# hypre-space/hypredrive

Hardware: AMD Instinct MI355X
Metric: DOF/s, AMG-PCG solve phase, 3D 7-pt Laplacian (higher is better)
Workload: dtype f64

## Files before the change

### hypredrive_amd/_lib.py

```python
import ctypes as C
import os

import numpy as np

_HERE = os.path.dirname(os.path.abspath(__file__))
_LIBPATH = os.path.join(_HERE, "lib", "libhypredrv_amd.so")
_L = None


class LibraryError(RuntimeError):
    pass


class AmgParams(C.Structure):
    _fields_ = [("coarsen_type", C.c_int), ("interp_type", C.c_int), ("pmax", C.c_int),
                ("trunc_factor", C.c_double), ("strong_th", C.c_double),
                ("max_row_sum", C.c_double), ("max_coarse_size", C.c_int),
                ("min_coarse_size", C.c_int), ("max_levels", C.c_int),
                ("relax_down", C.c_int), ("relax_up", C.c_int), ("relax_coarse", C.c_int),
                ("sweeps_down", C.c_int), ("sweeps_up", C.c_int), ("sweeps_coarse", C.c_int),
                ("relax_weight", C.c_double), ("outer_weight", C.c_double),
                ("seed", C.c_uint64), ("num_functions", C.c_int),
                ("cheby_order", C.c_int), ("cheby_eig_est", C.c_int), ("cheby_variant", C.c_int), ("cheby_scale", C.c_int),
                ("cheby_fraction", C.c_double),
# ... 94 lines not shown
        "hda_mgr_blk_inverses": (I, [VP, I, I, DP, IP, IP]),
        "hda_amg_num_levels": (I, [VP]), "hda_amg_level_matrix": (I, [VP, I, I, OUT]), "hda_amg_level_cf": (I, [VP, I, IP]),
        "hda_amg_fold_sweep": (I, [VP, I, DP, DP, DP, DP, DP]), "hda_amg_blocks": (I, [VP]), "hda_amg_level_blocks": (I, [VP, I, LP]),
        "hda_amg_complexities": (I, [VP, DP, DP]), "hda_amg_vcycle_bytes": (D, [VP]), "hda_amg_vcycle": (I, [VP, DP, DP]),
        "hda_pcg": krylov, "hda_gmres": krylov, "hda_fgmres": krylov, "hda_bicgstab": krylov,
        "hda_spmm": (I, [VP, I, I, D, D, DP, DP, DP, DP, DP, DP, DP]), "hda_multi_blas": (I, [I, I, I, DP, DP, IP, DP, DP, DP, DP, DP]),
        "hda_amg_vcycle_multi": (I, [VP, I, DP, DP]), "hda_pcg_multi": (I, [VP, VP, KRY, I, DP, DP, DP, IP, IP, DP]),
        "hda_time_kernel_multi": (I, [I, VP, VP, I, I, DP, DP]),
        "hda_time_kernel": (I, [I, VP, VP, I, DP, DP]), "hda_set_overlap": (None, [I]), "hda_last_precond_calls": (I, []),
        "hda_solve_device": (I, [VP, VP, KRY, I, DP, I, DP, IP, DP, DP, DP, DP]),
        "hda_pcg_iteration_bytes": (D, [VP]), "hda_format_bytes": (I, [VP, VP, DP, DP, DP, IP]),
        "hda_csr_form": (I, [VP, I, IP]), "hda_spmv_mode": (I, [VP, I, I, D, D, DP, DP, DP, DP, DP, DP, DP, DP, DP, IP]),
        "hda_borrow_hypredrv": (I, [VP, OUT, OUT]), "hda_amd_partitioned_levels": (I, [VP]), "hda_amd_hierarchy_levels": (I, [VP]),
        "hda_halo_plan_host": (I, [I, LLP, LLP, I, IP, IP, IP, I, IP]),
        "hda_dev_alloc": (I, [I64, OUT]), "hda_dev_free": (I, [VP]), "hda_dev_upload": (I, [VP, VP, I64]),
        "hda_dev_download": (I, [VP, VP, I64]), "hda_borrow_ij_matrix": (I, [VP, OUT]), "hda_ij_ghost_gids": (I, [VP, LLP, I, IP]),
        "hda_ij_last_assembly": (I, [DP]),
        "hda_probe_spmv": (I, [VP, I]), "hda_probe_read": (I, [DP, IP]), "hda_probe_add": (I, [VP, I, IP]),
        "hda_probe_read_id": (I, [I, DP, IP]),
        "hda_comm_stats": (I, [DP, I]), "hda_comm_name": (S, []), "hda_comm_size": (I, []), "hda_comm_selftest": (I, []),
        "hda_check_row_total": (I, [C.c_longlong, I]),
        "hda_memory_stats": (I, [DP, DP]), "hda_memory_cached": (D, []), "hda_memory_driver_stats": (I, [DP, I]), "hda_memory_trim": (I, []),
    }
    undeclared = {"hda_amg_rebind": (I, [VP, VP]), "hda_amg_level0_sweep": (I, [VP, I, DP, DP, DP, DP, IP])}
    return declared, undeclared


_DECLARED, _UNDECLARED = _signatures()
SYMBOLS = list(_DECLARED)


TESTRANKS_SYMBOLS = ["hda_thread_ranks_lap7", "hda_thread_world_create", "hda_thread_world_join", "hda_thread_world_leave",
                     "hda_thread_world_destroy", "hda_testranks_selftest"]
_TESTRANKS_PATH = os.path.join(os.path.dirname(_LIBPATH), "libhypredrv_amd_testranks.so")
_T = None


def load_testranks():
    global _T
    if _T is None:
        load()
        if not os.path.exists(_TESTRANKS_PATH):
            raise LibraryError(f"{_TESTRANKS_PATH} not built: run `python -c 'import __graft_entry__ as g; g.build()'`")
        _T = C.CDLL(_TESTRANKS_PATH)
    return _T


# ... 348 lines not shown
    def blocks(self):
        return load().hda_amg_blocks(self.h)

    def level_blocks(self, level):
        out = np.zeros(max(self.blocks, 1) + 1, dtype=np.int64)
        _check(load().hda_amg_level_blocks(self.h, level, out.ctypes.data_as(C.POINTER(C.c_int64))))
        return out

    @property
    def complexities(self):
        g, o = C.c_double(), C.c_double()
        _check(load().hda_amg_complexities(self.h, C.byref(g), C.byref(o)))
        return g.value, o.value

    @property
    def vcycle_bytes(self):
        return load().hda_amg_vcycle_bytes(self.h)

    def vcycle(self, b):
        b = np.ascontiguousarray(b, dtype=np.float64)
        x = np.zeros_like(b)
        _check(load().hda_amg_vcycle(self.h, _dp(b), _dp(x)))
        return x

    def vcycle_multi(self, B):
        B = _cols(B)
        k = B.shape[1]
        bt = np.ascontiguousarray(B.T)
        xt = np.zeros_like(bt)
        _check(load().hda_amg_vcycle_multi(self.h, k, _dp(bt), _dp(xt)))
        return xt.T.copy()


MGR_INTERP = {"injection": 0, "l1-jacobi": 1, "jacobi": 2, "blk-jacobi": 12}
MGR_COARSE = {"rap": 0, "galerkin": 0, "non-galerkin": 1}
MGR_RESTRICT = {"injection": 0, "jacobi": 2, "columped": 14}
MGR_FRELAX = {"jacobi": 7, "single": 7, "l1-jacobi": 18, "amg": 2, "ilu": 32}
MGR_GRELAX = {"none": -1, "h-fgs": 3, "h-bgs": 4, "h-ssor": 6, "l1-hfgs": 13, "l1-hbgs": 14, "l1-hsgs": 88, "ilu": 16}

MGR_KRYLOV = {"pcg": 1, "gmres": 2, "fgmres": 3, "bicgstab": 4}


def _mgr_nested(entry, lv):
    for key, pre in (("f_krylov", "frelax"), ("coarsest_krylov", "coarse")):
        nk = lv.get(key)
        if not nk:
# ... 585 lines not shown
```

### hypredrive_amd/csrc/hda_amg.h

```cpp
#pragma once

#include "hda_dist.h"
#include "hda_kernels.h"

#include <chrono>
#include <memory>
#include <string>
#include <vector>

namespace hda {

struct IluParams {
   int tri_solve = 1;
   int lower_it = 5, upper_it = 5;
   int max_iter = 1;
   int                    blocks = 1;
   std::vector<long long> block_part;
};

struct AmgParams {
   int    coarsen_type    = 8;
   double strong_th       = 0.25;
   double max_row_sum     = 0.9;
   int    max_coarse_size = 64;
// ... 180 lines not shown
 public:
   void        setup(const DCsr &A, const FsaiParams &p, const std::vector<int> *part = nullptr);
   void        apply(const double *r, double *z);
   const DCsr &factor() const { return G; }
   const DCsr &factor_t() const { return GT; }
   double      apply_bytes() const;
   FsaiParams  prm;
   int         n = 0, nblocks = 1, fallback_rows = 0;
   int         class_rows[5] = {0, 0, 0, 0, 0};
   double      omega = 1.0;
   double      setup_ms[4] = {0, 0, 0, 0};

 private:
   DCsr           G, GT;
   DArray<double> work;
};

struct FirstSweepFusion {
   bool          valid = false;
   const double *dinv  = nullptr;
   const unsigned char *rclass = nullptr;
   const double *cdinv = nullptr;
   double       *dest  = nullptr;
   int           n     = 0;
   const void   *owner = nullptr;
   bool          done  = false;
   const double *in    = nullptr;
   double       *out   = nullptr;
};
FirstSweepFusion &first_sweep_fusion();

struct AmgLevel {
   DCsr           A, P, R;
   DCsr           Pt;
   bool           folded = false;
   DCsr           Pg;
   bool           pg_ready = false;
   GsPlan         gs;
   std::unique_ptr<Ilu> ilu;
   std::unique_ptr<Fsai> fsai;
   bool complex_smoother() const { return ilu || fsai; }
   DArray<double> cheb_ds, cheb_v, cheb_w;
   double         cheb_coef[5] = {0, 0, 0, 0, 0}, cheb_max_eig = 0.0, cheb_min_eig = 0.0;
   DArray<double> ilu_r, ilu_c;
   DArray<int>    cf;
   std::vector<int> blk_part;
   DArray<double> dinv_down, dinv_up;
   DArray<double> cdinv_down, cdinv_up;
   unsigned long long cdinv_gen = 0;
   DArray<double> dinv_pts[2][2];
   TwoStage       ts;
// ... 29 lines not shown
   void apply(const double *b, double *x, int dot_slot = -1);
   void apply_offering(const double *b, double *x, int dot_slot = -1);
   bool first_sweep_fusable() const;
   double *first_sweep_dest(double *x);
   void solve(const double *b, double *x);
   void        apply_multi(const double *B, double *X, int K);
   std::string multi_cycle_refusal() const;
   double      vcycle_multi_bytes(int K) const;

   int           num_levels() const { return (int)levels.size(); }
   const DCsr   &level_A(int l) const { return l == 0 ? *A0 : levels[l].A; }
   AmgLevel     &level(int l) { return levels[l]; }
   double        operator_complexity() const;
   double        grid_complexity() const;
   double        vcycle_bytes(bool format = false) const;
   bool          level_folded(int l) const { return l >= 0 && l < num_levels() && levels[(size_t)l].folded; }
   bool          level0_sweep(int dir, const double *b, const double *x, double *out, int dot_slot);
   AmgParams     prm;
   int           blocks_used = 1;
   const std::vector<int> &level_blocks(int l) const { return levels[(size_t)l].blk_part; }
   double        setup_times[8] = {0};

 private:
   void cycle(const double *b, double *x, bool zero_guess, int dot_slot, bool first_sweep_given = false);
   void relax(int l, int type, const double *dinv, const double *b, double *&cur, double *&alt,
              bool zero_guess, int dot_slot);
   int           sweep_points(int dir, int s) const;
   const double *sweep_dinv(int l, int dir, int s);
   void          build_class_dinv();
   const double *class_dinv(int l, const double *dinv);
   void          check_air_params() const;
   bool          needs_cf_in_cycle() const;
   void build_hierarchy(const DCsr &A, bool keep_ap = false);
   void build_smoother_data(int l);
   bool fold_level(int l);
   void build_cheby(int l);
   void cheby_sweep(int l, const double *b, double *u, bool zero_guess, bool ghosts_fresh = false);
   bool ghosts_fresh_ = false;
   void coarse_solve(const double *f, double *u);
   const HaloPlan &level_hA(int l) const { return (l == 0 && hA0) ? *hA0 : levels[l].hA; }
   const DCsr           *A0 = nullptr;
   int                   a0_dims[3] = {0, 0, 0};
   const HaloPlan       *hA0 = nullptr;
   bool                  dist = false;
   long long             coarse_lo = 0;
   int                   coarse_nloc = 0;
   double                stats_nnz[32] = {0}, stats_rows[32] = {0};
// ... 192 lines not shown
```

### hypredrive_amd/csrc/hda_amg_setup.hip

```cpp
#include "hda_amg.h"
#include "hda_sort.h"


#include <algorithm>
#include <chrono>
#include <cstring>

namespace hda {

#define STREAM (Context::get().stream)

void exclusive_scan64(long n, const int *in, long long *out);


__global__ __launch_bounds__(256) void k_strength(int n, const int *__restrict__ rp,
                                                  const int *__restrict__ cj,
                                                  const double *__restrict__ v, double theta,
                                                  double mrs, unsigned char *__restrict__ smask,
                                                  int *__restrict__ ns, const int *__restrict__ dof)
{
   const int i = blockIdx.x * 256 + threadIdx.x;
   if (i >= n) return;
   const int k0 = rp[i], k1 = rp[i + 1];
   double    diag = 0.0, row_sum = 0.0, row_scale = 0.0;
// ... 3583 lines not shown

FirstSweepFusion &first_sweep_fusion()
{
   return RankState<FirstSweepFusion>::get();
}
bool Amg::first_sweep_fusable() const
{
   const char *e = getenv("HDA_FUSE_Z0");
   return !(e && atoi(e) == 0) && num_levels() > 1 && prm.sweeps_down >= 1 && is_jacobi_type(prm.relax_down) && !levels[0].complex_smoother();
}
double *Amg::first_sweep_dest(double *x)
{
   auto oop = [&](int t) { return is_jacobi_type(t) || (levels[0].gs.nblk > 0 && (t == 3 || t == 4 || t == 13 || t == 14)); };
   const int swaps0 = levels[0].complex_smoother() ? 0 : (oop(prm.relax_down) ? (prm.sweeps_down - (prm.sweeps_down > 0 ? 1 : 0)) : 0) +
                                             (oop(prm.relax_up) ? prm.sweeps_up : 0);
   return (swaps0 & 1) ? levels[0].u2.data() : x;
}
void Amg::apply_offering(const double *b, double *x, int dot_slot)
{
   FirstSweepFusion &fs = first_sweep_fusion();
   const bool given = fs.done && fs.owner == this && fs.in == b && fs.out == x;
   fs.done          = false;
   HDA_REQUIRE(!given || first_sweep_fusable(), "first sweep handed to a cycle that does not open with one");
   cycle(b, x, true, dot_slot, given);
   fs.valid = first_sweep_fusable();
   if (fs.valid)
   {
      double *d = first_sweep_dest(x);
      fs.dinv   = sweep_dinv(0, 0, 0);
      fs.cdinv  = class_dinv(0, fs.dinv);
      fs.rclass = fs.cdinv ? row_classes(level_A(0)) : nullptr;
      fs.dest   = (d == x) ? nullptr : d;
      fs.n      = level_A(0).nrows;
      fs.owner  = this;
   }
}

void Amg::cycle(const double *b, double *x, bool zero_guess, int dot_slot, bool first_sweep_given)
{
   const int L  = num_levels();
   const int n0 = level_A(0).nrows;
   for (AmgLevel &lv : levels) lv.gs_b_seen = false;
   if (L == 1)
   {
      if (coarse_dense) coarse_solve(b, x);
      else
      {
         double *cur = x, *alt = levels[0].u2.data();
         bool    zg  = zero_guess;
         for (int s = 0; s < std::max(prm.sweeps_coarse, 1); s++)
         {
            relax(0, prm.relax_coarse == 9 ? 18 : prm.relax_coarse, levels[0].dinv_down.data(), b, cur, alt, zg, -1);
            zg = false;
         }
         if (cur != x) copy(n0, cur, x);
      }
      if (dot_slot >= 0) dot(n0, b, x, dot_slot);
      return;
   }
   std::vector<double *> sol((size_t)L, nullptr);
   auto oop = [&](int t) { return is_jacobi_type(t) || (levels[0].gs.nblk > 0 && (t == 3 || t == 4 || t == 13 || t == 14)); };
// ... 8 lines not shown
   const bool fuse_first = !(getenv("HDA_FUSE_FIRST_SWEEP") && atoi(getenv("HDA_FUSE_FIRST_SWEEP")) == 0);
   const bool fold_up    = !(getenv("HDA_FOLD_UP") && atoi(getenv("HDA_FOLD_UP")) == 0);
   for (int l = 0; l < L - 1; l++)
   {
      const DCsr &A  = level_A(l);
      AmgLevel   &lv = levels[l];
      bool        zg = zero_guess || l > 0;
      if (zg && prm.sweeps_down == 0) fill(A.nrows, 0.0, cur);
      for (int s = 0; s < prm.sweeps_down; s++)
      {
         if (!(s == 0 && first_sweep_done)) relax(l, prm.relax_down, sweep_dinv(l, 0, s), f, cur, alt, zg, -1);
         zg = false;
      }
      residual(A, cur, f, lv.t.data(), &level_hA(l));
      AmgLevel &nx = levels[l + 1];
      first_sweep_done = false;
      if (fuse_first && l + 1 < L - 1 && prm.sweeps_down > 0 && is_jacobi_type(prm.relax_down) && !nx.complex_smoother())
         first_sweep_done = spmv_with_scaled_copy(lv.R, lv.t.data(), nx.f.data(), sweep_dinv(l + 1, 0, 0), nx.u.data(), &lv.hR);
      else
         spmv(lv.R, 1.0, lv.t.data(), 0.0, nullptr, nx.f.data(), &lv.hR);
      sol[l] = cur;
      f      = nx.f.data();
      if (l + 1 < L - 1) { cur = nx.u.data(); alt = nx.u2.data(); }
   }
   {
      AmgLevel &lc = levels[L - 1];
      if (coarse_dense) coarse_solve(lc.f.data(), lc.u.data());
      else
      {
         double *c2 = lc.u.data(), *a2 = lc.u2.data();
         bool    zg = true;
         for (int s = 0; s < std::max(prm.sweeps_coarse, 1); s++)
         {
            relax(L - 1, prm.relax_coarse == 9 ? 18 : prm.relax_coarse, lc.dinv_down.data(), lc.f.data(), c2, a2, zg, -1);
            zg = false;
         }
         if (c2 != lc.u.data()) copy(level_A(L - 1).nrows, c2, lc.u.data());
      }
      sol[L - 1] = lc.u.data();
   }
   for (int l = L - 2; l >= 0; l--)
   {
      AmgLevel &lv = levels[l];
      double   *c  = sol[l];
      double   *a;
      if (l == 0) a = (c == x) ? levels[0].u2.data() : x;
// ... 1118 lines not shown
```

### hypredrive_amd/csrc/hda_capi.hip

```cpp
#include "../../include/hypredrv_amd.h"

#include "hda_precond.h"
#include "hda_multi.h"
#include "hda_comm.h"
#include "hda_hypre.h"

#include <chrono>
#include <cmath>
#include <cstring>

using namespace hda;

struct hda_csr_s {
   DCsr           m;
   DArray<double> rhs;
   bool           borrowed = false;
   const DCsr    *ref      = nullptr;
   const double  *rhs_ref  = nullptr;
   const HaloPlan *halo    = nullptr;
   const DCsr    &get() const { return ref ? *ref : m; }
};
struct hda_amg_s {
   Precond                                 pc;
   hda_csr_t                               A = nullptr;
// ... 1033 lines not shown
   else for (size_t q = 0; q < bp.size(); q++) part[q] = bp[q];
   HDA_CATCH
}
extern "C" int hda_amg_complexities(hda_amg_t h, double *grid, double *op)
{
   if (!h) return HDA_ERR_ARG;
   if (grid) *grid = h->pc.amg->grid_complexity();
   if (op) *op = h->pc.amg->operator_complexity();
   return HDA_OK;
}
extern "C" double hda_amg_vcycle_bytes(hda_amg_t h) { return h ? h->pc.amg->vcycle_bytes() : 0.0; }

extern "C" int hda_amg_vcycle(hda_amg_t h, const double *b, double *x)
{
   HDA_TRY
   const DCsr    &m = h->pc.amg ? h->pc.amg->level_A(0) : h->A->get();
   DArray<double> db = staged(b, m.nrows), dx = room<double>(std::max((int)h->pc.vec_len(m), m.ncols));
   h->pc.solve(m, nullptr, db.data(), dx.data(), true);
   fetch(dx.data(), x, m.nrows);
   gs_free_check();
   HDA_CATCH
}


static int run_krylov(int kind, hda_csr_t A, hda_amg_t amg, const hda_krylov_params *kp, const double *b,
                      double *x, double *hist, int *iters, int *converged, double *final_rel)
{
   HDA_TRY
   const DCsr    &m = A->get();
   DArray<double> db = staged(b, m.nrows), dx = staged(x, m.nrows, m.ncols);
   PrecondFn      M;
   if (amg) M = amg->pc.as_fn(m, nullptr);
   KrylovParams  k   = to_kparams(kp);
   LinOp         op(m, nullptr, (amg && amg->pc.amg) ? amg->pc.amg->vec_len0() : 0);
   KrylovResult  res = kind == 1 ? gmres(op, M, k, db.data(), dx.data()) : kind == 2 ? fgmres(op, M, k, db.data(), dx.data())
                     : kind == 3 ? bicgstab(op, M, k, db.data(), dx.data()) : pcg(op, M, k, db.data(), dx.data());
   fetch(dx.data(), x, m.nrows);
   if (hist)
      for (size_t i = 0; i < res.hist.size() && i < (size_t)k.max_iter + 1; i++) hist[i] = res.hist[i];
   if (iters) *iters = res.iters;
   if (converged) *converged = res.converged ? 1 : 0;
   if (final_rel) *final_rel = res.final_rel;
   HDA_CATCH
}
extern "C" int hda_pcg(hda_csr_t A, hda_amg_t amg, const hda_krylov_params *kp, const double *b, double *x,
                       double *hist, int *iters, int *converged, double *final_rel)
// ... 228 lines not shown
   for (int w = 0; w < 3; w++) launch();
   hipEvent_t e0, e1;
   HDA_HIP(hipEventCreate(&e0));
   HDA_HIP(hipEventCreate(&e1));
   HDA_HIP(hipEventRecord(e0, ctx.stream));
   for (int r = 0; r < reps; r++) launch();
   HDA_HIP(hipEventRecord(e1, ctx.stream));
   HDA_HIP(hipEventSynchronize(e1));
   float ms = 0.f;
   HDA_HIP(hipEventElapsedTime(&ms, e0, e1));
   (void)hipEventDestroy(e0);
   (void)hipEventDestroy(e1);
   if (avg_ms) *avg_ms = (double)ms / std::max(reps, 1);
   if (bytes)
   {
      const double sb = spmv_alg_bytes(m);
      *bytes = (kind == 0) ? sb : (kind == 1) ? sb + 16.0 * m.nrows : (kind == 2) ? sb + 8.0 * m.nrows : amg->pc.amg->vcycle_bytes();
   }
   HDA_CATCH
}

extern "C" void hda_set_overlap(int mode) { set_overlap_mode(mode); }
extern "C" int hda_last_precond_calls(void) { return last_precond_calls(); }

extern "C" int hda_solve_device(hda_csr_t A, hda_amg_t amg, const hda_krylov_params *kp, int solver,
                                const double *b_host, int nsolves, double *solve_ms, int *iters,
                                double *final_rel, double *r0_norm, double *true_rel, double *k1_avg_ms)
{
   HDA_TRY
   using clk        = std::chrono::steady_clock;
   Context       &ctx = Context::get();
   const DCsr    &m   = A->get();
   const int      n   = m.nrows;
   DArray<double> b, x(std::max<size_t>((size_t)std::max(m.ncols, 1), amg && amg->pc.amg ? amg->pc.amg->vec_len0() : 0)), r((size_t)std::max(n, 1));
   if (b_host) b.upload(b_host, (size_t)n);
   else if (A->rhs_ref)
   {
      b.alloc((size_t)std::max(n, 1));
      copy(n, A->rhs_ref, b.data());
   }
   else
   {
      HDA_REQUIRE(A->rhs.size() == (size_t)n, "no right-hand side: pass b or build A with hda_lap7_create");
      b.copy_from(A->rhs);
   }
   x.zero();
// ... 322 lines not shown
```

### hypredrive_amd/csrc/hda_common.h

```cpp
#pragma once

#include <hip/hip_runtime.h>

#include <atomic>
#include <cstdint>
#include <cstdio>
#include <cstdlib>
#include <chrono>
#include <memory>
#include <stdexcept>
#include <string>
#include <utility>
#include <vector>

namespace hda {

struct Error : std::runtime_error {
   using std::runtime_error::runtime_error;
};

#define HDA_HIP(expr)                                                                    \
   do {                                                                                  \
      hipError_t _e = (expr);                                                            \
      if (_e != hipSuccess)                                                              \
// ... 49 lines not shown
   {
      delete mine_;
      mine_ = nullptr;
   }
   static thread_local T *mine_;
};
template <class T, int Tag>
thread_local T *RankState<T, Tag>::mine_ = nullptr;

void        wait_stream(hipStream_t s);
void        wait_event(hipEvent_t e);
double      wait_limit_s();
void        set_stage(const char *stage);
const char *current_stage();
[[noreturn]] void abort_job(int status);

struct Context {
   hipStream_t stream      = nullptr;
   hipStream_t comm_stream = nullptr;
   double     *partials    = nullptr;
   double     *scalars     = nullptr;
   double     *host_scalars = nullptr;
   hipEvent_t  ev           = nullptr;
   int         device       = 0;
   static constexpr int kNumSlots   = 8;
   static constexpr int kNumScalars = 320;

   static Context &get();
   static void     release_thread();
   void            sync() { wait_stream(stream); }
   double         *slot(int s) { return partials + (size_t)s * kRedBlocks; }

 private:
   Context();
};

void *pool_alloc(size_t bytes);
void  pool_free(void *p);
void  pool_trim();
size_t pool_bytes_in_use();
size_t pool_bytes_peak();
size_t pool_bytes_cached();
void   pool_driver_stats(double out[3], bool reset);

template <class T>
class DArray {
// ... 146 lines not shown
```

### hypredrive_amd/csrc/hda_kernels.h

```cpp
#pragma once

#include "hda_common.h"

namespace hda {

struct HaloPlan;


void spmv(const DCsr &A, double alpha, const double *x, double beta, const double *y_in,
          double *y_out, const HaloPlan *halo = nullptr);
bool spmv_with_scaled_copy(const DCsr &A, const double *x, double *y, const double *dinv2, double *y2, const HaloPlan *halo = nullptr);
void spmv_dot(const DCsr &A, const double *x, double *y, const double *w, int slot, const HaloPlan *halo = nullptr);
void residual(const DCsr &A, const double *x, const double *b, double *out, const HaloPlan *halo = nullptr);

void jacobi(const DCsr &A, const double *dinv, const double *b, const double *x_in,
            double *x_out, int dot_slot, const HaloPlan *halo = nullptr, const double *cdinv = nullptr);
bool class_divisors(const DCsr &A, const double *dinv, DArray<double> &table);
const unsigned char *row_classes(const DCsr &A);
void jacobi_folded(const DCsr &A, const DCsr &Pt, const double *dinv, const double *t, const double *e, const double *u, double *out);
bool spmv_foldable(const DCsr &Pt);
void jacobi_zero_guess(int n, const double *dinv, const double *b, double *x);

enum Scalar : int {
   S_GAMMA0 = 0, S_RR0 = 1, S_GAMMA1 = 2, S_RR1 = 3, S_SP = 4, S_BB = 5, S_TMP = 6, S_TMP2 = 7,
   S_GMRES = 8
};
void dot(int n, const double *x, const double *y, int slot);
void finalize(int slot, int scalar_idx);
void finalize_n(int first_slot, int nslots, int first_scalar);
void cg_update(int n, int gamma_idx, const double *p, const double *s, double *x, double *r, int rr_slot, int sp_slot = -1,
               const double *dinv0 = nullptr, double *z0 = nullptr, const unsigned char *rclass = nullptr, const double *cdinv = nullptr);
void cg_direction(int n, int gamma_old_idx, int gamma_new_idx, const double *z, double *p, int first_slot = -1, double *x = nullptr);
void cg_flush_x(int n, int gamma_idx, const double *p, double *x);
void cg_single_step(int n, int t_new, int t_old, int alpha_idx, bool first, const double *u, const double *w, double *p, double *s, double *x,
                    double *r, int rr_slot);
void axpy(int n, double a, const double *x, double *y);
void axpy_dev(int n, int scalar_idx, double sign, const double *x, double *y);
void scale(int n, double a, double *x);
void scale_inv_sqrt_dev(int n, int scalar_idx, double *x);
void copy(int n, const double *x, double *y);
void fill(int n, double v, double *x);
void mul(int n, const double *a, const double *b, double *out);
double read_scalar(int idx);
void   read_scalars_async(int first, int count);

void dense_apply(int n, const double *inv, const double *b, double *x);
void dense_invert(int n, double *a, double *inv);
void csr_to_dense(const DCsr &A, double *dense);

void exclusive_scan(int n, const int *in, int *out, int *total_out_dev);
void require_int32_total(long n, const int *counts, const char *what);
void l1_row_norms(const DCsr &A, int option, double *l1, const int *part = nullptr, int nb = 0);
void extract_diag(const DCsr &A, double *d);
void make_dinv(int n, const double *d, double weight, double *dinv);
double matrix_stream_bytes(const DCsr &A, bool format);
double rowptr_stream_bytes(const DCsr &A, bool format);
// ... 30 lines not shown
```

### hypredrive_amd/csrc/hda_kernels.hip

```cpp
#include "hda_kernels.h"
#include "hda_sort.h"

#include "hda_dist.h"
#include "hda_mpi_join.h"
#include <unistd.h>

#include <algorithm>
#include <cmath>
#include <cstring>
#include <limits>
#include <map>
#include <mutex>
#include <type_traits>
#include <unordered_map>
#include <rocprim/device/device_segmented_radix_sort.hpp>

namespace hda {


Context::Context()
{
   HDA_HIP(hipGetDevice(&device));
   HDA_HIP(hipStreamCreateWithFlags(&stream, hipStreamNonBlocking));
   {
      int lo = 0, hi = 0;
      if (hipDeviceGetStreamPriorityRange(&lo, &hi) != hipSuccess) { (void)hipGetLastError(); hi = 0; }
      if (hipStreamCreateWithPriority(&comm_stream, hipStreamNonBlocking, hi) != hipSuccess)
      {
         (void)hipGetLastError();
         HDA_HIP(hipStreamCreateWithFlags(&comm_stream, hipStreamNonBlocking));
      }
   }
   HDA_HIP(hipMalloc((void **)&partials, sizeof(double) * kNumSlots * kRedBlocks));
   HDA_HIP(hipMemset(partials, 0, sizeof(double) * kNumSlots * kRedBlocks));
   HDA_HIP(hipMalloc((void **)&scalars, sizeof(double) * kNumScalars));
   HDA_HIP(hipMemset(scalars, 0, sizeof(double) * kNumScalars));
   HDA_HIP(hipHostMalloc((void **)&host_scalars, sizeof(double) * kNumScalars, hipHostMallocDefault));
   HDA_HIP(hipEventCreateWithFlags(&ev, hipEventDisableTiming));
}

namespace {
const char *g_stage_name = "idle";
template <class Query>
void wait_limited(Query done, const char *what)
{
   const double lim = wait_limit_s();
   const auto   t0  = std::chrono::steady_clock::now();
   for (long spin = 0;; spin++)
   {
      hipError_t e = done();
      if (e == hipSuccess) return;
      if (e != hipErrorNotReady) HDA_HIP(e);
      (void)hipGetLastError();
      if (spin > 2000) usleep(20);
      if (std::chrono::duration<double>(std::chrono::steady_clock::now() - t0).count() > lim)
      {
         fprintf(stderr, "[hypredrv_amd] rank %d of %d (%s transport): a %s wait did not end within %.1f s (HDA_COMM_TIMEOUT_S) during %s: a peer "
                         "rank has failed or left the collective sequence, or a kernel hangs; ending the job\n", Comm::world().rank, Comm::world().size,
                 Comm::world().name(), what, lim, g_stage_name);
         abort_job(86);
      }
   }
// ... 50 lines not shown
      tl_drops = nullptr;
   }
   delete tl_ctx;
   tl_ctx  = nullptr;
   tl_rank = false;
}

Context &Context::get()
{
   if (!tl_rank)
   {
      static Context ctx;
      return ctx;
   }
   if (!tl_ctx) tl_ctx = new Context();
   return *tl_ctx;
}
void Context::release_thread()
{
   if (!tl_rank || !tl_ctx) return;
   Context &c = get();
   (void)hipStreamSynchronize(c.stream);
   (void)hipStreamSynchronize(c.comm_stream);
   pool_trim();
   (void)hipFree(c.partials); (void)hipFree(c.scalars); (void)hipHostFree(c.host_scalars);
   (void)hipEventDestroy(c.ev); (void)hipStreamDestroy(c.comm_stream); (void)hipStreamDestroy(c.stream);
   c.partials = c.scalars = c.host_scalars = nullptr; c.ev = nullptr; c.stream = c.comm_stream = nullptr;
}


namespace {
struct Cached {
   void    *p;
   uint64_t stamp;
};
struct Pool;
std::mutex                          g_pool_mutex;
std::unordered_map<void *, Pool *> &block_owner()
{
   static std::unordered_map<void *, Pool *> m;
   return m;
}
std::vector<Pool *> &all_pools()
{
   static std::vector<Pool *> v;
   return v;
// ... 2423 lines not shown
   if (first_slot >= 0)
   {
      const int g = std::max(ew_grid(n), 1);
      if (x) k_cg_dir<true, true><<<g, 256, 0, STREAM>>>(n, c.scalars, gamma_old_idx, gamma_new_idx, z, p, c.slot(first_slot), x);
      else k_cg_dir<true, false><<<g, 256, 0, STREAM>>>(n, c.scalars, gamma_old_idx, gamma_new_idx, z, p, c.slot(first_slot), nullptr);
   }
   else if (n)
   {
      if (x) k_cg_dir<false, true><<<ew_grid(n), 256, 0, STREAM>>>(n, c.scalars, gamma_old_idx, gamma_new_idx, z, p, nullptr, x);
      else k_cg_dir<false, false><<<ew_grid(n), 256, 0, STREAM>>>(n, c.scalars, gamma_old_idx, gamma_new_idx, z, p, nullptr, nullptr);
   }
}

__global__ __launch_bounds__(256) void k_cg_flush_x(int n, const double *__restrict__ scalars, int gamma_idx, const double *__restrict__ p,
                                                    double *__restrict__ x)
{
   const double alpha = scalars[gamma_idx] / scalars[S_SP];
   for (long i = (long)blockIdx.x * 256 + threadIdx.x; i < n; i += (long)gridDim.x * 256) x[i] += alpha * p[i];
}
void cg_flush_x(int n, int gamma_idx, const double *p, double *x)
{
   if (n) k_cg_flush_x<<<ew_grid(n), 256, 0, STREAM>>>(n, Context::get().scalars, gamma_idx, p, x);
}

__global__ __launch_bounds__(256) void k_cg_single(int n, double *scalars, int t_new, int t_old, int alpha_idx, int first, const double *__restrict__ u,
                                                   const double *__restrict__ w, double *__restrict__ p, double *__restrict__ s,
                                                   double *__restrict__ x, double *__restrict__ r, double *__restrict__ partial)
{
   const double gn = scalars[t_new], delta = scalars[t_new + 2];
   double       beta = 0.0, alpha;
   if (first) alpha = gn / delta;
   else
   {
      beta  = gn / scalars[t_old];
      alpha = gn / (delta - beta * gn / scalars[alpha_idx]);
   }
   double acc = 0.0;
   for (long i = (long)blockIdx.x * 256 + threadIdx.x; i < n; i += (long)gridDim.x * 256)
   {
      const double pi = u[i] + beta * p[i], si = w[i] + beta * s[i];
      p[i]            = pi;
      s[i]            = si;
      x[i] += alpha * pi;
      const double ri = r[i] - alpha * si;
      r[i]            = ri;
      acc += ri * ri;
// ... 655 lines not shown
```

### hypredrive_amd/csrc/hda_krylov.h

```cpp
#pragma once

#include "hda_amg.h"

#include <functional>
#include <limits>

namespace hda {

struct KrylovParams {
   int    max_iter    = 100;
   double rtol        = 1.0e-6;
   double atol        = 0.0;
   int    two_norm    = 1;
   int    print_level = 0;
   int    krylov_dim  = 30;
   int    min_iter    = 0;
   int    skip_real_res_check = 0;
   bool   profile_k1 = false;
};

struct KrylovResult {
   int                 iters     = 0;
   bool                converged = false;
   double              final_rel = 0.0;
// ... 5 lines not shown

using PrecondFn = std::function<void(const double *r, double *z, int dot_slot)>;

struct LinOp {
   const DCsr     *A      = nullptr;
   const HaloPlan *halo   = nullptr;
   size_t          veclen = 0;
   LinOp() = default;
   LinOp(const DCsr &a) : A(&a), veclen((size_t)std::max(a.ncols, a.nrows)) {}
   LinOp(const DCsr &a, const HaloPlan *h, size_t len) : A(&a), halo(h), veclen(std::max(len, (size_t)std::max(a.ncols, a.nrows))) {}
};

struct PcgKnown {
   bool   x_zero = false;
   double bb     = std::numeric_limits<double>::quiet_NaN();
};

KrylovResult pcg(const LinOp &op, const PrecondFn &M, const KrylovParams &p, const double *b, double *x, const PcgKnown *known = nullptr);
KrylovResult gmres(const LinOp &op, const PrecondFn &M, const KrylovParams &p, const double *b, double *x);
KrylovResult fgmres(const LinOp &op, const PrecondFn &M, const KrylovParams &p, const double *b, double *x);
KrylovResult bicgstab(const LinOp &op, const PrecondFn &M, const KrylovParams &p, const double *b, double *x);

int    last_precond_calls();
double pcg_iteration_bytes(const DCsr &A, bool format = false);

}
```

### hypredrive_amd/csrc/hda_krylov.hip

```cpp
#include "hda_krylov.h"

#include <cmath>

namespace hda {

#define g_last_precond_calls (RankState<int, 5>::get())
int last_precond_calls() { return g_last_precond_calls; }

namespace {
struct NestedScope {
   static thread_local int depth;
   DArray<double>          save;
   bool                    nested;
   static constexpr size_t kScal = Context::kNumScalars, kPart = (size_t)Context::kNumSlots * kRedBlocks;
   NestedScope() : nested(depth++ > 0)
   {
      if (!nested) return;
      Context &ctx = Context::get();
      save.alloc(kScal + kPart);
      HDA_HIP(hipMemcpyAsync(save.data(), ctx.scalars, kScal * sizeof(double), hipMemcpyDeviceToDevice, ctx.stream));
      HDA_HIP(hipMemcpyAsync(save.data() + kScal, ctx.partials, kPart * sizeof(double), hipMemcpyDeviceToDevice, ctx.stream));
   }
   ~NestedScope()
   {
      depth--;
      if (!nested) return;
      Context &ctx = Context::get();
      (void)hipMemcpyAsync(ctx.scalars, save.data(), kScal * sizeof(double), hipMemcpyDeviceToDevice, ctx.stream);
      (void)hipMemcpyAsync(ctx.partials, save.data() + kScal, kPart * sizeof(double), hipMemcpyDeviceToDevice, ctx.stream);
   }
};
thread_local int NestedScope::depth = 0;
}

double pcg_iteration_bytes(const DCsr &A, bool format)
{
   const double n = A.nrows;
   const char  *dxe = getenv("HDA_DEFER_X");
   const double vec = (format && !(dxe && atoi(dxe) == 0)) ? 24.0 * n + 40.0 * n : 48.0 * n + 24.0 * n;
   return (matrix_stream_bytes(A, format) + rowptr_stream_bytes(A, format) + 8.0 * A.ncols + 8.0 * n) + 8.0 * n + vec;
}

static KrylovResult pcg_single_reduction(const LinOp &op, const PrecondFn &M, const KrylovParams &kp, const double *b, double *x)
{
   Context     &ctx = Context::get();
   const DCsr  &A   = *op.A;
   const int    n   = A.nrows;
   KrylovResult res;
   const size_t vl = std::max<size_t>(op.veclen, 1);
   DArray<double> r(vl), u(vl), w(vl), p(vl), s(vl);
   constexpr int T0 = S_GMRES, T1 = S_GMRES + 3, S_ALPHA = S_GMRES + 6;
   auto precond = [&](const double *rr, double *zz, int slot) {
      res.precond_calls++;
      if (M) M(rr, zz, slot);
      else
      {
         copy(n, rr, zz);
         if (slot >= 0) dot(n, rr, zz, slot);
      }
   };
   dot(n, b, b, 0);
   finalize(0, S_BB);
// ... 75 lines not shown
      if (sr && atoi(sr) != 0)
      {
         KrylovResult r1 = pcg_single_reduction(op, M, kp, b, x);
         g_last_precond_calls = r1.precond_calls;
         return r1;
      }
   }
   Context     &ctx = Context::get();
   const DCsr  &A   = *op.A;
   const int    n   = A.nrows;
   KrylovResult res;
   const size_t vl = std::max<size_t>(op.veclen, 1);
   DArray<double> r(vl), p(vl), s(vl);

   FirstSweepFusion &fs = first_sweep_fusion();
   fs                   = FirstSweepFusion();
   struct FsReset {
      ~FsReset() { first_sweep_fusion() = FirstSweepFusion(); }
   } fs_reset;
   const double *z0_dinv = nullptr, *z0_cdinv = nullptr;
   const unsigned char *z0_rclass = nullptr;
   double       *z0_dest = nullptr;
   bool          z0_self = false;
   auto precond = [&](const double *rr, double *zz, int slot) {
      res.precond_calls++;
      fs.valid = false;
      if (M) M(rr, zz, slot);
      else
      {
         copy(n, rr, zz);
         if (slot >= 0) dot(n, rr, zz, slot);
      }
      HDA_REQUIRE(!fs.done, "the preconditioner ignored a first sweep it had offered to take from the caller");
      const bool mine = fs.valid && fs.n == n;
      z0_dinv = mine ? fs.dinv : nullptr;
      z0_dest = mine ? fs.dest : nullptr;
      z0_cdinv  = mine ? fs.cdinv : nullptr;
      z0_rclass = mine ? fs.rclass : nullptr;
      z0_self = mine && fs.dest == nullptr;
      fs.valid = false;
   };
   const char *ffe = getenv("HDA_FUSE_FINALIZE");
   const int   fl  = (Comm::world().size == 1) ? (ffe ? atoi(ffe) : 1) : 0;
   const bool  fin = fl >= 1, fin2 = fl >= 2;
   const char *dxe     = getenv("HDA_DEFER_X");
   const bool  defer_x = !(dxe && atoi(dxe) == 0);
   double     *xd      = defer_x ? x : nullptr;

   double bi_prod;
   if (kp.two_norm && known && !std::isnan(known->bb)) bi_prod = known->bb;
   else
   {
      if (kp.two_norm) dot(n, b, b, 0);
      else precond(b, p.data(), 0);
      finalize(0, S_BB);
      bi_prod = read_scalar(S_BB);
   }
   if (bi_prod == 0.0)
   {
      copy(n, b, x);
      ctx.sync();
      res.hist.push_back(0.0);
      return res;
   }
   double eps = kp.rtol * kp.rtol;
   {
      const double a2 = kp.atol * kp.atol / bi_prod;
      if (a2 > eps) eps = a2;
   }
   if (known && known->x_zero) copy(n, b, r.data());
   else
   {
      copy(n, x, p.data());
      residual(A, p.data(), b, r.data(), op.halo);
   }
   precond(r.data(), p.data(), 2);
   dot(n, r.data(), r.data(), 3);
   finalize_n(2, 2, S_GAMMA0);
   read_scalars_async(S_GAMMA0, 5);
   wait_event(ctx.ev);
   double i_prod = kp.two_norm ? ctx.host_scalars[S_RR0] : ctx.host_scalars[S_GAMMA0];
   res.hist.push_back(std::sqrt(std::fabs(i_prod)));
   int it = 0, x_term = -1;
   std::vector<hipEvent_t> evs;
   static const bool fuse_dots = !(getenv("HDA_FUSE_DOTS") && atoi(getenv("HDA_FUSE_DOTS")) == 0);
   while (it + 1 <= kp.max_iter)
   {
      it++;
      const int go = (it & 1) ? S_GAMMA0 : S_GAMMA1, gn = (it & 1) ? S_GAMMA1 : S_GAMMA0, rn = gn + 1;
      if (kp.profile_k1)
      {
         hipEvent_t e0, e1;
         HDA_HIP(hipEventCreate(&e0));
         HDA_HIP(hipEventCreate(&e1));
         HDA_HIP(hipEventRecord(e0, ctx.stream));
         spmv_dot(A, p.data(), s.data(), p.data(), 0, op.halo);
         HDA_HIP(hipEventRecord(e1, ctx.stream));
         evs.push_back(e0);
         evs.push_back(e1);
      }
      else
         spmv_dot(A, p.data(), s.data(), p.data(), 0, op.halo);
      if (!fin) finalize(0, S_SP);
      double *z0 = z0_dinv ? (z0_self ? s.data() : z0_dest) : nullptr;
      cg_update(n, go, p.data(), s.data(), defer_x ? nullptr : x, r.data(), 3, fin ? 0 : -1, z0_dinv, z0, z0_rclass, z0_cdinv);
      x_term = defer_x ? go : -1;
      bool stop = false;
      auto test = [&]() {
         wait_event(ctx.ev);
         const double sp = ctx.host_scalars[S_SP];
         if (sp == 0.0 || !std::isfinite(sp))
         {
            it--;
            stop = true;
            return;
         }
         i_prod = kp.two_norm ? ctx.host_scalars[rn] : ctx.host_scalars[gn];
         res.hist.push_back(std::sqrt(std::fabs(i_prod)));
         if (kp.print_level >= 2)
            printf("%5d    %e    %f    %e\n", it, res.hist.back(),
                   res.hist[res.hist.size() - 2] > 0 ? res.hist.back() / res.hist[res.hist.size() - 2] : 0.0,
                   std::sqrt(i_prod / bi_prod));
         if (i_prod / bi_prod < eps)
         {
            res.converged = true;
            stop          = true;
         }
      };
      bool near = false;
      if (kp.two_norm && res.hist.size() >= 2)
      {
         const double h1 = res.hist.back(), h0 = res.hist[res.hist.size() - 2];
         const double rho2 = (h0 > 0.0) ? (h1 / h0) * (h1 / h0) : 1.0;
         near = h1 * h1 * rho2 < 16.0 * eps * bi_prod;
      }
      if (near)
      {
         finalize(3, rn);
         read_scalars_async(S_GAMMA0, 5);
         test();
         if (stop) break;
         fs.done = z0 != nullptr;
         fs.in   = r.data();
         fs.out  = s.data();
         precond(r.data(), s.data(), 2);
         if (fin2) cg_direction(n, go, gn, s.data(), p.data(), 2, xd);
         else
         {
            finalize(2, gn);
            cg_direction(n, go, gn, s.data(), p.data(), -1, xd);
         }
         x_term = -1;
         continue;
      }
      if (!fuse_dots) finalize(3, rn);
      fs.done = z0 != nullptr;
      fs.in   = r.data();
      fs.out  = s.data();
      precond(r.data(), s.data(), 2);
      if (fin2 && fuse_dots)
      {
         cg_direction(n, go, gn, s.data(), p.data(), 2, xd);
         read_scalars_async(S_GAMMA0, 5);
      }
      else
      {
         if (fuse_dots) finalize_n(2, 2, gn);
         else finalize(2, gn);
         read_scalars_async(S_GAMMA0, 5);
         cg_direction(n, go, gn, s.data(), p.data(), -1, xd);
      }
      x_term = -1;
      test();
      if (stop) break;
   }
   fs = FirstSweepFusion();
   if (x_term >= 0) cg_flush_x(n, x_term, p.data(), x);
   ctx.sync();
   gs_free_check();
   for (size_t e = 0; e + 1 < evs.size(); e += 2)
   {
      float ms = 0.f;
      if (hipEventElapsedTime(&ms, evs[e], evs[e + 1]) == hipSuccess)
      {
         res.k1_ms_sum += ms;
         res.k1_count++;
      }
      (void)hipEventDestroy(evs[e]);
      (void)hipEventDestroy(evs[e + 1]);
   }
   res.iters     = it;
   res.final_rel = std::sqrt(std::fabs(i_prod) / bi_prod);
   if (!scope.nested) g_last_precond_calls = res.precond_calls;
   return res;
}

static KrylovResult gmres_core(bool flexible, const LinOp &op, const PrecondFn &M, const KrylovParams &kp, const double *b, double *x)
{
   NestedScope  scope;
   Context     &ctx = Context::get();
   const DCsr  &A   = *op.A;
   const int    n = A.nrows, k = std::max(kp.krylov_dim, 1);
   KrylovResult res;
   HDA_REQUIRE(S_GMRES + k + 2 <= Context::kNumScalars, "krylov_dim too large for the scalar block");
   const size_t vlen = std::max<size_t>(op.veclen, 1);
   std::vector<DArray<double>> V((size_t)k + 1);
   for (auto &v : V) v.alloc(vlen);
   DArray<double> w(vlen), r(vlen);
   std::vector<DArray<double>> Z(flexible ? (size_t)k : 0);
   for (auto &z : Z) z.alloc(vlen);
   auto true_residual = [&](double *out) {
      copy(n, x, w.data());
      residual(A, w.data(), b, out, op.halo);
   };
   std::vector<double> H((size_t)(k + 1) * k, 0.0), cs((size_t)k), sn((size_t)k), rs((size_t)k + 1);

// ... 194 lines not shown
```

Baseline: 604.3 million.

## Overlap deferred x update on side stream during coarse V-cycle levels

Adds an optional side stream that runs the deferred PCG x update concurrently with the coarse part of the AMG V-cycle. The V-cycle records an event after restriction reaches a coarse level, and the x flush then runs there with a limited grid before joining the main stream. The goal is to hide the bandwidth cost of the x update behind the latency-bound coarse levels. Separately, when enabled by default, the SpMV output is placed into the first-sweep destination buffer (shared z0), which changes buffer traffic. This adds stream and event synchronization and contention risk.

```diff
diff --git a/hypredrive_amd/_lib.py b/hypredrive_amd/_lib.py
--- a/hypredrive_amd/_lib.py
+++ b/hypredrive_amd/_lib.py
@@ -140,7 +140,8 @@
         "hda_check_row_total": (I, [C.c_longlong, I]),
         "hda_memory_stats": (I, [DP, DP]), "hda_memory_cached": (D, []), "hda_memory_driver_stats": (I, [DP, I]), "hda_memory_trim": (I, []),
     }
-    undeclared = {"hda_amg_rebind": (I, [VP, VP]), "hda_amg_level0_sweep": (I, [VP, I, DP, DP, DP, DP, IP])}
+    undeclared = {"hda_amg_rebind": (I, [VP, VP]), "hda_amg_level0_sweep": (I, [VP, I, DP, DP, DP, DP, IP]),
+                  "hda_amg_vcycle_offered": (I, [VP, DP, DP, IP]), "hda_last_side_passes": (I, [])}
     return declared, undeclared
 
 
@@ -535,6 +536,12 @@
         x = np.zeros_like(b)
         _check(load().hda_amg_vcycle(self.h, _dp(b), _dp(x)))
         return x
+
+    def vcycle_offered(self, b):
+        b = np.ascontiguousarray(b, dtype=np.float64)
+        x, where = np.zeros_like(b), C.c_int()
+        _check(load().hda_amg_vcycle_offered(self.h, _dp(b), _dp(x), C.byref(where)))
+        return x, where.value
 
     def vcycle_multi(self, B):
         B = _cols(B)
diff --git a/hypredrive_amd/csrc/hda_amg.h b/hypredrive_amd/csrc/hda_amg.h
--- a/hypredrive_amd/csrc/hda_amg.h
+++ b/hypredrive_amd/csrc/hda_amg.h
@@ -226,11 +226,14 @@
    const unsigned char *rclass = nullptr;
    const double *cdinv = nullptr;
    double       *dest  = nullptr;
+   bool          share = false;
    int           n     = 0;
    const void   *owner = nullptr;
    bool          done  = false;
    const double *in    = nullptr;
    double       *out   = nullptr;
+   hipEvent_t    mark   = nullptr;
+   bool          marked = false;
 };
 FirstSweepFusion &first_sweep_fusion();
 
@@ -306,7 +309,7 @@
    double        setup_times[8] = {0};
 
  private:
-   void cycle(const double *b, double *x, bool zero_guess, int dot_slot, bool first_sweep_given = false);
+   void cycle(const double *b, double *x, bool zero_guess, int dot_slot, bool first_sweep_given = false, hipEvent_t mark = nullptr);
    void relax(int l, int type, const double *dinv, const double *b, double *&cur, double *&alt,
               bool zero_guess, int dot_slot);
    int           sweep_points(int dir, int s) const;
diff --git a/hypredrive_amd/csrc/hda_amg_setup.hip b/hypredrive_amd/csrc/hda_amg_setup.hip
--- a/hypredrive_amd/csrc/hda_amg_setup.hip
+++ b/hypredrive_amd/csrc/hda_amg_setup.hip
@@ -3629,7 +3629,10 @@
    const bool given = fs.done && fs.owner == this && fs.in == b && fs.out == x;
    fs.done          = false;
    HDA_REQUIRE(!given || first_sweep_fusable(), "first sweep handed to a cycle that does not open with one");
-   cycle(b, x, true, dot_slot, given);
+   hipEvent_t mark = fs.mark;
+   fs.mark         = nullptr;
+   fs.marked       = false;
+   cycle(b, x, true, dot_slot, given, mark);
    fs.valid = first_sweep_fusable();
    if (fs.valid)
    {
@@ -3638,12 +3641,14 @@
       fs.cdinv  = class_dinv(0, fs.dinv);
       fs.rclass = fs.cdinv ? row_classes(level_A(0)) : nullptr;
       fs.dest   = (d == x) ? nullptr : d;
+      const char *zs = getenv("HDA_Z0_IN_S");
+      fs.share       = fs.dest && !(zs && atoi(zs) == 0);
       fs.n      = level_A(0).nrows;
       fs.owner  = this;
    }
 }
 
-void Amg::cycle(const double *b, double *x, bool zero_guess, int dot_slot, bool first_sweep_given)
+void Amg::cycle(const double *b, double *x, bool zero_guess, int dot_slot, bool first_sweep_given, hipEvent_t mark)
 {
    const int L  = num_levels();
    const int n0 = level_A(0).nrows;
@@ -3698,6 +3703,12 @@
       sol[l] = cur;
       f      = nx.f.data();
       if (l + 1 < L - 1) { cur = nx.u.data(); alt = nx.u2.data(); }
+      if (mark && (l == 1 || l == L - 2))
+      {
+         HDA_HIP(hipEventRecord(mark, STREAM));
+         first_sweep_fusion().marked = true;
+         mark                        = nullptr;
+      }
    }
    {
       AmgLevel &lc = levels[L - 1];
diff --git a/hypredrive_amd/csrc/hda_capi.hip b/hypredrive_amd/csrc/hda_capi.hip
--- a/hypredrive_amd/csrc/hda_capi.hip
+++ b/hypredrive_amd/csrc/hda_capi.hip
@@ -1079,6 +1079,34 @@
    HDA_CATCH
 }
 
+extern "C" int hda_amg_vcycle_offered(hda_amg_t h, const double *b, double *x, int *where)
+{
+   HDA_TRY
+   HDA_REQUIRE(h && h->pc.amg && b && x && where, "hda_amg_vcycle_offered: null argument");
+   Amg              &amg = *h->pc.amg;
+   const DCsr       &m   = amg.level_A(0);
+   DArray<double>    db = staged(b, m.nrows), dx = room<double>(std::max((int)h->pc.vec_len(m), m.ncols));
+   FirstSweepFusion &fs = first_sweep_fusion();
+   fs                   = FirstSweepFusion();
+   amg.apply_offering(db.data(), dx.data(), -1);
+   *where = !fs.valid ? 0 : !fs.dest ? 1 : fs.share ? 3 : 2;
+   if (fs.valid)
+   {
+      double *d = fs.dest ? fs.dest : dx.data();
+      if (fs.dest) fill(m.nrows, std::numeric_limits<double>::quiet_NaN(), dx.data());
+      if (fs.dest && fs.share) fill(m.nrows, std::numeric_limits<double>::quiet_NaN(), d);
+      mul(m.nrows, fs.dinv, db.data(), d);
+      fs.done = true;
+      fs.in   = db.data();
+      fs.out  = dx.data();
+   }
+   amg.apply_offering(db.data(), dx.data(), -1);
+   fs = FirstSweepFusion();
+   fetch(dx.data(), x, m.nrows);
+   gs_free_check();
+   HDA_CATCH
+}
+
 
 static int run_krylov(int kind, hda_csr_t A, hda_amg_t amg, const hda_krylov_params *kp, const double *b,
                       double *x, double *hist, int *iters, int *converged, double *final_rel)
@@ -1353,6 +1381,7 @@
 
 extern "C" void hda_set_overlap(int mode) { set_overlap_mode(mode); }
 extern "C" int hda_last_precond_calls(void) { return last_precond_calls(); }
+extern "C" int hda_last_side_passes(void) { return last_side_passes(); }
 
 extern "C" int hda_solve_device(hda_csr_t A, hda_amg_t amg, const hda_krylov_params *kp, int solver,
                                 const double *b_host, int nsolves, double *solve_ms, int *iters,
diff --git a/hypredrive_amd/csrc/hda_common.h b/hypredrive_amd/csrc/hda_common.h
--- a/hypredrive_amd/csrc/hda_common.h
+++ b/hypredrive_amd/csrc/hda_common.h
@@ -95,6 +95,9 @@
    double     *scalars     = nullptr;
    double     *host_scalars = nullptr;
    hipEvent_t  ev           = nullptr;
+   hipStream_t side_stream = nullptr;
+   hipEvent_t  side_mark = nullptr, side_done = nullptr;
+   void        need_side();
    int         device       = 0;
    static constexpr int kNumSlots   = 8;
    static constexpr int kNumScalars = 320;
diff --git a/hypredrive_amd/csrc/hda_kernels.h b/hypredrive_amd/csrc/hda_kernels.h
--- a/hypredrive_amd/csrc/hda_kernels.h
+++ b/hypredrive_amd/csrc/hda_kernels.h
@@ -32,6 +32,9 @@
                const double *dinv0 = nullptr, double *z0 = nullptr, const unsigned char *rclass = nullptr, const double *cdinv = nullptr);
 void cg_direction(int n, int gamma_old_idx, int gamma_new_idx, const double *z, double *p, int first_slot = -1, double *x = nullptr);
 void cg_flush_x(int n, int gamma_idx, const double *p, double *x);
+constexpr int kSideGrid = 256;
+void cg_flush_x_side(int n, int gamma_idx, const double *p, double *x, int grid);
+void cg_side_join();
 void cg_single_step(int n, int t_new, int t_old, int alpha_idx, bool first, const double *u, const double *w, double *p, double *s, double *x,
                     double *r, int rr_slot);
 void axpy(int n, double a, const double *x, double *y);
diff --git a/hypredrive_amd/csrc/hda_kernels.hip b/hypredrive_amd/csrc/hda_kernels.hip
--- a/hypredrive_amd/csrc/hda_kernels.hip
+++ b/hypredrive_amd/csrc/hda_kernels.hip
@@ -38,6 +38,13 @@
    HDA_HIP(hipHostMalloc((void **)&host_scalars, sizeof(double) * kNumScalars, hipHostMallocDefault));
    HDA_HIP(hipEventCreateWithFlags(&ev, hipEventDisableTiming));
 }
+void Context::need_side()
+{
+   if (side_stream) return;
+   HDA_HIP(hipStreamCreateWithFlags(&side_stream, hipStreamNonBlocking));
+   HDA_HIP(hipEventCreateWithFlags(&side_mark, hipEventDisableTiming));
+   HDA_HIP(hipEventCreateWithFlags(&side_done, hipEventDisableTiming));
+}
 
 namespace {
 const char *g_stage_name = "idle";
@@ -134,6 +141,12 @@
    Context &c = get();
    (void)hipStreamSynchronize(c.stream);
    (void)hipStreamSynchronize(c.comm_stream);
+   if (c.side_stream)
+   {
+      (void)hipStreamSynchronize(c.side_stream);
+      (void)hipEventDestroy(c.side_mark); (void)hipEventDestroy(c.side_done); (void)hipStreamDestroy(c.side_stream);
+      c.side_stream = nullptr; c.side_mark = c.side_done = nullptr;
+   }
    pool_trim();
    (void)hipFree(c.partials); (void)hipFree(c.scalars); (void)hipHostFree(c.host_scalars);
    (void)hipEventDestroy(c.ev); (void)hipStreamDestroy(c.comm_stream); (void)hipStreamDestroy(c.stream);
@@ -2603,6 +2616,19 @@
 {
    if (n) k_cg_flush_x<<<ew_grid(n), 256, 0, STREAM>>>(n, Context::get().scalars, gamma_idx, p, x);
 }
+void cg_flush_x_side(int n, int gamma_idx, const double *p, double *x, int grid)
+{
+   Context &c = Context::get();
+   HDA_REQUIRE(c.side_stream && grid >= 1, "side pass: no side stream");
+   HDA_HIP(hipStreamWaitEvent(c.side_stream, c.side_mark, 0));
+   if (n) k_cg_flush_x<<<std::min(grid, ew_grid(n)), 256, 0, c.side_stream>>>(n, c.scalars, gamma_idx, p, x);
+   HDA_HIP(hipEventRecord(c.side_done, c.side_stream));
+}
+void cg_side_join()
+{
+   Context &c = Context::get();
+   HDA_HIP(hipStreamWaitEvent(c.stream, c.side_done, 0));
+}
 
 __global__ __launch_bounds__(256) void k_cg_single(int n, double *scalars, int t_new, int t_old, int alpha_idx, int first, const double *__restrict__ u,
                                                    const double *__restrict__ w, double *__restrict__ p, double *__restrict__ s,
diff --git a/hypredrive_amd/csrc/hda_krylov.h b/hypredrive_amd/csrc/hda_krylov.h
--- a/hypredrive_amd/csrc/hda_krylov.h
+++ b/hypredrive_amd/csrc/hda_krylov.h
@@ -51,6 +51,7 @@
 KrylovResult bicgstab(const LinOp &op, const PrecondFn &M, const KrylovParams &p, const double *b, double *x);
 
 int    last_precond_calls();
+int    last_side_passes();
 double pcg_iteration_bytes(const DCsr &A, bool format = false);
 
 }
diff --git a/hypredrive_amd/csrc/hda_krylov.hip b/hypredrive_amd/csrc/hda_krylov.hip
--- a/hypredrive_amd/csrc/hda_krylov.hip
+++ b/hypredrive_amd/csrc/hda_krylov.hip
@@ -1,21 +1,26 @@
 #include "hda_krylov.h"
 
 #include <cmath>
+#include <cstring>
 
 namespace hda {
 
 #define g_last_precond_calls (RankState<int, 5>::get())
 int last_precond_calls() { return g_last_precond_calls; }
+#define g_last_side_passes (RankState<int, 6>::get())
+int last_side_passes() { return g_last_side_passes; }
 
 namespace {
 struct NestedScope {
    static thread_local int depth;
+   static thread_local long entries;
    DArray<double>          save;
    bool                    nested;
    static constexpr size_t kScal = Context::kNumScalars, kPart = (size_t)Context::kNumSlots * kRedBlocks;
    NestedScope() : nested(depth++ > 0)
    {
       if (!nested) return;
+      entries++;
       Context &ctx = Context::get();
       save.alloc(kScal + kPart);
       HDA_HIP(hipMemcpyAsync(save.data(), ctx.scalars, kScal * sizeof(double), hipMemcpyDeviceToDevice, ctx.stream));
@@ -31,13 +36,21 @@
    }
 };
 thread_local int NestedScope::depth = 0;
+thread_local long NestedScope::entries = 0;
+}
+
+static bool x_place_side()
+{
+   const char *e = getenv("HDA_X_PLACE");
+   return e && strcmp(e, "side") == 0 && Comm::world().size == 1;
 }
 
 double pcg_iteration_bytes(const DCsr &A, bool format)
 {
    const double n = A.nrows;
-   const char  *dxe = getenv("HDA_DEFER_X");
-   const double vec = (format && !(dxe && atoi(dxe) == 0)) ? 24.0 * n + 40.0 * n : 48.0 * n + 24.0 * n;
+   const char  *dxe  = getenv("HDA_DEFER_X");
+   const bool   side = x_place_side();
+   const double vec  = (format && !(dxe && atoi(dxe) == 0)) ? 24.0 * n + (side ? 48.0 : 40.0) * n : 48.0 * n + 24.0 * n;
    return (matrix_stream_bytes(A, format) + rowptr_stream_bytes(A, format) + 8.0 * A.ncols + 8.0 * n) + 8.0 * n + vec;
 }
 
@@ -159,6 +172,7 @@
    const unsigned char *z0_rclass = nullptr;
    double       *z0_dest = nullptr;
    bool          z0_self = false;
+   bool          z0_share = false;
    auto precond = [&](const double *rr, double *zz, int slot) {
       res.precond_calls++;
       fs.valid = false;
@@ -175,6 +189,7 @@
       z0_cdinv  = mine ? fs.cdinv : nullptr;
       z0_rclass = mine ? fs.rclass : nullptr;
       z0_self = mine && fs.dest == nullptr;
+      z0_share = mine && fs.dest && fs.share && Comm::world().size == 1;
       fs.valid = false;
    };
    const char *ffe = getenv("HDA_FUSE_FINALIZE");
@@ -183,6 +198,23 @@
    const char *dxe     = getenv("HDA_DEFER_X");
    const bool  defer_x = !(dxe && atoi(dxe) == 0);
    double     *xd      = defer_x ? x : nullptr;
+   const bool  x_side    = defer_x && !scope.nested && x_place_side();
+   const char *xge       = getenv("HDA_X_SIDE_GRID");
+   const int   side_grid = (xge && atoi(xge) > 0) ? atoi(xge) : kSideGrid;
+   int side_passes = 0;
+   if (x_side) ctx.need_side();
+   auto precond_x = [&](int go) -> double * {
+      const long nested0 = NestedScope::entries;
+      if (x_side) { fs.mark = ctx.side_mark; fs.marked = false; }
+      precond(r.data(), s.data(), 2);
+      const bool marked = x_side && fs.marked && nested0 == NestedScope::entries;
+      fs.mark = nullptr;
+      fs.marked = false;
+      if (!marked) return xd;
+      cg_flush_x_side(n, go, p.data(), x, side_grid);
+      side_passes++;
+      return nullptr;
+   };
 
    double bi_prod;
    if (kp.two_norm && known && !std::isnan(known->bb)) bi_prod = known->bb;
@@ -225,22 +257,23 @@
    {
       it++;
       const int go = (it & 1) ? S_GAMMA0 : S_GAMMA1, gn = (it & 1) ? S_GAMMA1 : S_GAMMA0, rn = gn + 1;
+      double *sv = (z0_dinv && z0_share) ? z0_dest : s.data();
       if (kp.profile_k1)
       {
          hipEvent_t e0, e1;
          HDA_HIP(hipEventCreate(&e0));
          HDA_HIP(hipEventCreate(&e1));
          HDA_HIP(hipEventRecord(e0, ctx.stream));
-         spmv_dot(A, p.data(), s.data(), p.data(), 0, op.halo);
+         spmv_dot(A, p.data(), sv, p.data(), 0, op.halo);
          HDA_HIP(hipEventRecord(e1, ctx.stream));
          evs.push_back(e0);
          evs.push_back(e1);
       }
       else
-         spmv_dot(A, p.data(), s.data(), p.data(), 0, op.halo);
+         spmv_dot(A, p.data(), sv, p.data(), 0, op.halo);
       if (!fin) finalize(0, S_SP);
       double *z0 = z0_dinv ? (z0_self ? s.data() : z0_dest) : nullptr;
-      cg_update(n, go, p.data(), s.data(), defer_x ? nullptr : x, r.data(), 3, fin ? 0 : -1, z0_dinv, z0, z0_rclass, z0_cdinv);
+      cg_update(n, go, p.data(), sv, defer_x ? nullptr : x, r.data(), 3, fin ? 0 : -1, z0_dinv, z0, z0_rclass, z0_cdinv);
       x_term = defer_x ? go : -1;
       bool stop = false;
       auto test = [&]() {
@@ -280,12 +313,13 @@
          fs.done = z0 != nullptr;
          fs.in   = r.data();
          fs.out  = s.data();
-         precond(r.data(), s.data(), 2);
-         if (fin2) cg_direction(n, go, gn, s.data(), p.data(), 2, xd);
+         double *xn = precond_x(go);
+         if (!xn && xd) cg_side_join();
+         if (fin2) cg_direction(n, go, gn, s.data(), p.data(), 2, xn);
          else
          {
             finalize(2, gn);
-            cg_direction(n, go, gn, s.data(), p.data(), -1, xd);
+            cg_direction(n, go, gn, s.data(), p.data(), -1, xn);
          }
          x_term = -1;
          continue;
@@ -294,10 +328,11 @@
       fs.done = z0 != nullptr;
       fs.in   = r.data();
       fs.out  = s.data();
-      precond(r.data(), s.data(), 2);
+      double *xn = precond_x(go);
       if (fin2 && fuse_dots)
       {
-         cg_direction(n, go, gn, s.data(), p.data(), 2, xd);
+         if (!xn && xd) cg_side_join();
+         cg_direction(n, go, gn, s.data(), p.data(), 2, xn);
          read_scalars_async(S_GAMMA0, 5);
       }
       else
@@ -305,7 +340,8 @@
          if (fuse_dots) finalize_n(2, 2, gn);
          else finalize(2, gn);
          read_scalars_async(S_GAMMA0, 5);
-         cg_direction(n, go, gn, s.data(), p.data(), -1, xd);
+         if (!xn && xd) cg_side_join();
+         cg_direction(n, go, gn, s.data(), p.data(), -1, xn);
       }
       x_term = -1;
       test();
@@ -329,6 +365,7 @@
    res.iters     = it;
    res.final_rel = std::sqrt(std::fabs(i_prod) / bi_prod);
    if (!scope.nested) g_last_precond_calls = res.precond_calls;
+   if (!scope.nested) g_last_side_passes = side_passes;
    return res;
 }
 
```

Result: no change. 604.8 million (median of 3 runs) (+0.1%).
